# ZenHKD/ocr-vi-invoice

Hardware: AMD Instinct MI355X
Metric: invoice images/sec end-to-end (det+rec) (higher is better)
Workload: dtype f16x2

## Files before the change

include/ocrvi.h:

```cpp
#ifndef OCRVI_H
#define OCRVI_H

#include <stddef.h>
#include <stdint.h>

#ifdef __cplusplus
extern "C" {
#endif

#define OCRVI_OK 0
#define OCRVI_EINVAL (-1)
#define OCRVI_EHIP (-2)
#define OCRVI_ENOMEM (-3)
#define OCRVI_EBLOB (-4)
#define OCRVI_ERANGE (-5)

typedef enum { OCRVI_F32 = 0, OCRVI_BF16 = 1, OCRVI_F16 = 2, OCRVI_F16X2 = 3 } ocrvi_dtype;

const char* ocrvi_last_error(void);
int ocrvi_abi_version(void);

typedef struct ocrvi_det ocrvi_det;

typedef struct {
// ... 262 lines not shown
                        int C, int H, int W, int Co, int ksize, int sh, int sw, int groups, int act, int res_post, int out_f32, int in_place,
                        void* out_raw, float* out);
int ocrvi_test_gconv_plan(int dtype, int N, int C, int H, int W, int Co, int sh, int sw, int groups, int out_f32, int has_res, int n_cu,
                          int32_t plan[12]);
int ocrvi_test_conv3_halo_raw(int device, const float* x, const float* weight_host, const float* bias_host, int N, int C, int H, int W, int Co,
                              int act, void* out_raw, float* out);
int ocrvi_test_bneck_tail_raw(int device, const float* t1, const float* identity, const float* w2_host, const float* b2_host,
                              const float* w3_host, const float* b3_host, const float* w1_host, const float* b1_host, int N, int H, int W,
                              int no_phase_c, void* y_raw, void* t1n_raw, float* y_out, float* t1n_out);
int ocrvi_test_stem_pool_raw(int device, int dtype, const float* x, const float* weight_host, const float* bias_host, int N, int H, int W,
                             int fused, void* out_raw, float* out);
int ocrvi_test_halo_plan(int kind, int N, int C, int H, int W, int Co, int n_cu, int32_t plan[8]);
int ocrvi_test_stem_pool(int device, int dtype, const float* x, const float* weight_host, const float* bias_host, int N, int H, int W, int fused,
                         float* out, int iters, float* avg_ms);
int ocrvi_test_attention(int device, int dtype, const float* qkv, int B, int N, int heads, float* out, int iters,
                         float* avg_ms);

int ocrvi_test_mlp(int device, int dtype, float* x, const float* ln_g_host, const float* ln_b_host, const float* w1_host, const float* b1_host,
                   const float* w2_host, const float* b2_host, const float* next_g_host, const float* next_b_host, int want_xn, int M, int D,
                   float* xn_out, int iters, float* avg_ms);
int ocrvi_test_mlp_raw(int device, int dtype, float* x, const float* ln_g_host, const float* ln_b_host, const float* w1_host, const float* b1_host,
                       const float* w2_host, const float* b2_host, const float* next_g_host, const float* next_b_host, int M, int D, void* xn_raw,
                       float* xn_out, int iters, float* avg_ms);
int ocrvi_test_lin_x2(int device, const float* a, const float* weight_host, const float* bias_host, int M, int K, int N, int max_workgroups,
                      void* out_raw, float* out, int iters, float* avg_ms);
int ocrvi_test_pack_f16x2(const float* src, size_t n, void* dst, float* wscale);
int ocrvi_test_pack_stream(int kind, const float* w0, const float* w1, int d0, int d1, void* out, size_t cap, size_t* size, float scales[2]);
int ocrvi_test_swizzles(int32_t swz128_rows[64], int32_t swz_halo_rows[64]);
int ocrvi_test_persistent_grid(int ntile, int slots, int32_t* grid);

int ocrvi_test_layernorm(int device, int dtype, const float* x, int x_f32, int out_f32, const float* gamma_host, const float* beta_host,
                         int rows, int D, float* out);
int ocrvi_test_frm_vertical(int device, int dtype, const float* kv, const float* vq_host, int B, int H, int W, int D, float* out);
int ocrvi_test_asf(int device, int dtype, const float* p2, const float* p3, const float* p4, const float* p5, const float* w_host,
                   const float* b_host, int N, int H, int W, float* out);
int ocrvi_test_maxpool(int device, int dtype, const float* x, int N, int C, int H, int W, float* out);
int ocrvi_test_db_maps(int device, const float* bin_logits, const float* thresh_logits, float k, float* binary, float* thresh,
                       float* thresh_binary, size_t n);
int ocrvi_test_ctc_logsoftmax(int device, const float* logits, int ld, int B, int T, int C, float* log_probs, int32_t* argmax_ids);
int ocrvi_test_ctc_logsoftmax_conf(int device, const float* logits, int ld, int B, int T, int C, float* log_probs, int32_t* argmax_ids,
                                   float* best_lp);

int ocrvi_document_contour(const uint8_t* mask, int h, int w, int64_t stride, int32_t* quad , int32_t* found);
int ocrvi_document_contour_bits(const uint32_t* bits, int h, int w, int32_t* quad , int32_t* found);

#define OCRVI_DOC_AUTO 0
// ... 21 lines not shown
```

ocr_vi_invoice_amd/_lib.py:

```python
from __future__ import annotations

import ctypes as C
import os
from typing import Optional

_HERE = os.path.dirname(os.path.abspath(__file__))
LIB_PATH = os.environ.get("OCRVI_LIB") or os.path.join(_HERE, "lib", "libocrvi.so")

OCRVI_F32, OCRVI_BF16, OCRVI_F16, OCRVI_F16X2 = 0, 1, 2, 3
DTYPES = {"f32": OCRVI_F32, "fp32": OCRVI_F32, "float32": OCRVI_F32, "bf16": OCRVI_BF16, "bfloat16": OCRVI_BF16,
          "f16": OCRVI_F16, "fp16": OCRVI_F16, "float16": OCRVI_F16,
          "f16x2": OCRVI_F16X2}
ABI_VERSION = 5

EXPORTS = [
    "ocrvi_last_error", "ocrvi_abi_version",
    "ocrvi_det_create", "ocrvi_det_destroy", "ocrvi_det_workspace_bytes", "ocrvi_det_forward", "ocrvi_det_debug_features",
    "ocrvi_rec_create", "ocrvi_rec_destroy", "ocrvi_rec_workspace_bytes", "ocrvi_rec_forward", "ocrvi_rec_debug_features",
    "ocrvi_ctc_greedy", "ocrvi_normalize_u8", "ocrvi_resize_u8", "ocrvi_crop_resize_normalize", "ocrvi_db_postprocess", "ocrvi_db_boxes_batch",
    "ocrvi_unclip_polygon", "ocrvi_db_components_workspace_bytes", "ocrvi_db_components", "ocrvi_db_boxes_batch_sparse",
    "ocrvi_test_deform_conv", "ocrvi_test_offset_conv", "ocrvi_test_conv", "ocrvi_test_gemm", "ocrvi_test_attention", "ocrvi_test_mlp", "ocrvi_test_stem_pool", "ocrvi_test_pack_f16x2",
    "ocrvi_prof_enable", "ocrvi_prof_reset", "ocrvi_prof_report",
    "ocrvi_det_status", "ocrvi_rec_status", "ocrvi_range_reset", "ocrvi_range_flag",
    "ocrvi_resize_normalize_pages", "ocrvi_crop_resize_normalize_pages", "ocrvi_db_boxes_pages",
    "ocrvi_det_binary_workspace_bytes", "ocrvi_det_forward_binary",
    "ocrvi_four_point_transform", "ocrvi_warp_perspective_u8", "ocrvi_warp_perspective_pages",
    "ocrvi_test_layernorm", "ocrvi_test_frm_vertical", "ocrvi_test_asf", "ocrvi_test_maxpool", "ocrvi_test_db_maps", "ocrvi_test_ctc_logsoftmax",
    "ocrvi_det_eval_workspace_bytes", "ocrvi_det_eval", "ocrvi_ctc_loss", "ocrvi_edit_distance",
    "ocrvi_test_deform_conv_res",
    "ocrvi_enhance_init", "ocrvi_enhance_tables", "ocrvi_enhance_workspace_bytes", "ocrvi_enhance_u8",
    "ocrvi_rgb_to_lab_u8", "ocrvi_lab_to_rgb_u8", "ocrvi_clahe_lab_u8", "ocrvi_nlm_lab_u8", "ocrvi_sharpen_u8",
    "ocrvi_min_area_quads", "ocrvi_quad_crops", "ocrvi_crop_quad_resize_normalize_pages", "ocrvi_crop_quad_resize_normalize",
    "ocrvi_jpeg_info", "ocrvi_jpeg_parse", "ocrvi_jpeg_table_entry", "ocrvi_jpeg_decode_pages",
    "ocrvi_test_conv_res", "ocrvi_test_db_tail",
    "ocrvi_db_target_jobs", "ocrvi_db_target_maps", "ocrvi_resize_normalize_pad_pages",
    "ocrvi_test_mlp_raw", "ocrvi_test_lin_x2", "ocrvi_test_pack_stream", "ocrvi_test_swizzles", "ocrvi_test_persistent_grid",
    "ocrvi_test_bneck_tail",
    "ocrvi_jpeg_quant_tables", "ocrvi_jpeg_encode_header", "ocrvi_jpeg_encode_sizes", "ocrvi_jpeg_encode_table_entry", "ocrvi_jpeg_encode_pages",
    "ocrvi_test_gemm_raw", "ocrvi_test_ring_plan",
    "ocrvi_overlay_segments", "ocrvi_overlay_pages",
    "ocrvi_test_deform_conv_raw", "ocrvi_test_dcn_plan",
    "ocrvi_test_conv_raw", "ocrvi_test_gconv_plan",
    "ocrvi_png_info", "ocrvi_png_parse", "ocrvi_png_table_entry", "ocrvi_png_plan", "ocrvi_png_decode_pages",
    "ocrvi_png_encode_sizes", "ocrvi_png_encode_table_entry", "ocrvi_png_encode_pages", "ocrvi_test_png_code_lengths",
    "ocrvi_document_contour", "ocrvi_document_contour_bits", "ocrvi_doc_working_size", "ocrvi_doc_mask_sizes", "ocrvi_doc_mask_pages",
    "ocrvi_doc_grey_u8", "ocrvi_doc_smooth_u8", "ocrvi_doc_histogram", "ocrvi_doc_otsu", "ocrvi_doc_mask_bits",
    "ocrvi_rec_forward_conf", "ocrvi_ctc_greedy_conf", "ocrvi_test_ctc_logsoftmax_conf",
    "ocrvi_test_conv3_halo_raw", "ocrvi_test_bneck_tail_raw", "ocrvi_test_stem_pool_raw", "ocrvi_test_halo_plan",
    "ocrvi_ctc_beam_workspace_bytes", "ocrvi_ctc_beam",
]
PAGE_ENTRY = 4
DET_EVAL_RECORD_BYTES = 104
DET_EVAL_INT_SLOTS = ("tp", "fp", "fn", "positive_count", "negatives", "negative_count")
DET_EVAL_F64_SLOTS = ("pos_bce", "topk_bce", "dice_inter", "pred_mask", "gt_mask", "l1_num", "thresh_mask")
CTC_LOSS_MAX_TARGET = 1024
EDIT_DISTANCE_MAX_LEN = 2048
CTC_BEAM_MAX = 64
CTC_BEAM_MAX_T = 1024
CLAHE_WORKSPACE_BYTES = 16384
# ... 99 lines not shown
    lib.ocrvi_test_offset_conv.argtypes = [i32, i32, f32p, vp, vp, i32, i32, i32, i32, i32, f32p, i32, C.POINTER(C.c_float)]
    lib.ocrvi_test_conv.argtypes = [i32, i32, f32p, vp, vp, i32, i32, i32, i32, i32, i32, i32, i32, i32, i32, f32p, i32,
                                    C.POINTER(C.c_float)]
    lib.ocrvi_test_conv_res.argtypes = [i32, i32, f32p, vp, vp, f32p, i32, i32, i32, i32, i32, i32, i32, i32, f32p, i32, C.POINTER(C.c_float)]
    lib.ocrvi_test_bneck_tail.argtypes = [i32, f32p, f32p, vp, vp, vp, vp, vp, vp, i32, i32, i32, i32, f32p, f32p, i32, C.POINTER(C.c_float)]
    lib.ocrvi_test_db_tail.argtypes = [i32, i32, f32p, vp, vp, vp, vp, vp, vp, vp, vp, i32, i32, i32, i32, i32, f32p, f32p, i32,
                                       C.POINTER(C.c_float)]
    lib.ocrvi_test_gemm.argtypes = [i32, i32, f32p, vp, vp, f32p, i32, i32, i32, i32, i32, i32, f32p, i32, C.POINTER(C.c_float)]
    lib.ocrvi_test_gemm_raw.argtypes = [i32, i32, f32p, vp, vp, f32p, i32, i32, i32, i32, i32, i32, vp, f32p]
    lib.ocrvi_test_ring_plan.argtypes = [i32, i32, i32, i32, i32, i32, i32, i32, C.POINTER(C.c_int32)]
    lib.ocrvi_test_deform_conv_raw.argtypes = [i32, i32, f32p, f32p, f32p, vp, vp, f32p, i32, i32, i32, i32, i32, i32, i32, vp, f32p]
    lib.ocrvi_test_dcn_plan.argtypes = [i32, i32, i32, i32, i32, i32, i32, i32, C.POINTER(C.c_int32)]
    lib.ocrvi_test_conv_raw.argtypes = [i32, i32, f32p, vp, vp, f32p] + [i32] * 13 + [vp, f32p]
    lib.ocrvi_test_gconv_plan.argtypes = [i32] * 12 + [C.POINTER(C.c_int32)]
    lib.ocrvi_test_stem_pool.argtypes = [i32, i32, f32p, vp, vp, i32, i32, i32, i32, f32p, i32, C.POINTER(C.c_float)]
    lib.ocrvi_test_conv3_halo_raw.argtypes = [i32, f32p, vp, vp, i32, i32, i32, i32, i32, i32, vp, f32p]
    lib.ocrvi_test_bneck_tail_raw.argtypes = [i32, f32p, f32p, vp, vp, vp, vp, vp, vp, i32, i32, i32, i32, vp, vp, f32p, f32p]
    lib.ocrvi_test_stem_pool_raw.argtypes = [i32, i32, f32p, vp, vp, i32, i32, i32, i32, vp, f32p]
    lib.ocrvi_test_halo_plan.argtypes = [i32] * 7 + [C.POINTER(C.c_int32)]
    lib.ocrvi_test_attention.argtypes = [i32, i32, f32p, i32, i32, i32, f32p, i32, C.POINTER(C.c_float)]
    lib.ocrvi_test_mlp.argtypes = [i32, i32, f32p, vp, vp, vp, vp, vp, vp, vp, vp, i32, i32, i32, f32p, i32, C.POINTER(C.c_float)]
    lib.ocrvi_test_lin_x2.argtypes = [i32, f32p, vp, vp, i32, i32, i32, i32, vp, f32p, i32, C.POINTER(C.c_float)]
    lib.ocrvi_test_mlp_raw.argtypes = [i32, i32, f32p, vp, vp, vp, vp, vp, vp, vp, vp, i32, i32, vp, f32p, i32, C.POINTER(C.c_float)]
    lib.ocrvi_test_pack_f16x2.argtypes = [f32p, sz, vp, C.POINTER(C.c_float)]
    lib.ocrvi_test_pack_stream.argtypes = [i32, vp, vp, i32, i32, vp, sz, C.POINTER(sz), C.POINTER(C.c_float)]
    lib.ocrvi_test_swizzles.argtypes = [C.POINTER(C.c_int32), C.POINTER(C.c_int32)]
    lib.ocrvi_test_persistent_grid.argtypes = [i32, i32, C.POINTER(C.c_int32)]
    lib.ocrvi_test_layernorm.argtypes = [i32, i32, f32p, i32, i32, vp, vp, i32, i32, f32p]
    lib.ocrvi_test_frm_vertical.argtypes = [i32, i32, f32p, vp, i32, i32, i32, i32, f32p]
    lib.ocrvi_test_asf.argtypes = [i32, i32, f32p, f32p, f32p, f32p, vp, vp, i32, i32, i32, f32p]
    lib.ocrvi_test_maxpool.argtypes = [i32, i32, f32p, i32, i32, i32, i32, f32p]
    lib.ocrvi_test_db_maps.argtypes = [i32, f32p, f32p, C.c_float, f32p, f32p, f32p, sz]
    lib.ocrvi_test_ctc_logsoftmax.argtypes = [i32, f32p, i32, i32, i32, i32, f32p, i32p]
    lib.ocrvi_det_eval_workspace_bytes.argtypes = [i32, i32, i32, C.POINTER(sz)]
    lib.ocrvi_det_eval.argtypes = [i32, f32p, f32p, f32p, f32p, f32p, f32p, f32p, f32p, i32, i32, i32, C.c_double, vp, vp, sz, vp]
    lib.ocrvi_ctc_loss.argtypes = [i32, f32p, i32, i32, i32, i32p, i32, i32p, i32p, i32, vp, vp]
    lib.ocrvi_edit_distance.argtypes = [i32, i32p, i32, i32p, i32p, i32, i32p, i32, i32p, vp]
    lib.ocrvi_ctc_beam_workspace_bytes.argtypes = [i32, i32, i32, i32, C.POINTER(sz)]
    lib.ocrvi_ctc_beam.argtypes = [i32, f32p, i32, i32, i32, i32, i32, i32, i32p, i32p, vp, vp, sz, vp]
    lib.ocrvi_enhance_init.argtypes = [i32]
    lib.ocrvi_enhance_tables.argtypes = [vp, sz, C.POINTER(sz)]
    lib.ocrvi_enhance_workspace_bytes.argtypes = [i32, i32, C.POINTER(sz)]
    lib.ocrvi_enhance_u8.argtypes = [i32, vp, i32, i32, vp, vp, sz, vp]
    for name in ("ocrvi_rgb_to_lab_u8", "ocrvi_lab_to_rgb_u8", "ocrvi_nlm_lab_u8", "ocrvi_sharpen_u8"):
        getattr(lib, name).argtypes = [i32, vp, i32, i32, vp, vp]
    lib.ocrvi_clahe_lab_u8.argtypes = [i32, vp, i32, i32, vp, vp, sz, vp]
# ... 92 lines not shown
```

ocr_vi_invoice_amd/csrc/gemm_ring.h:

```cpp
#pragma once
#include "conv_gemm.h"

namespace ocrvi {

__device__ __forceinline__ void glds16(const char* sbase, unsigned voff, unsigned lds_dst) {
    unsigned keep;
    asm volatile("s_mov_b32 %0, m0\n\ts_mov_b32 m0, %3\n\ts_nop 0\n\tglobal_load_lds_dwordx4 %1, %2\n\ts_mov_b32 m0, %0"
                 : "=&s"(keep)
                 : "v"(voff), "s"(sbase), "s"(lds_dst)
                 : "memory");
}
__device__ __forceinline__ void glds16_sc1(const char* sbase, unsigned voff, unsigned lds_dst) {
    unsigned keep;
    asm volatile("s_mov_b32 %0, m0\n\ts_mov_b32 m0, %3\n\ts_nop 0\n\tglobal_load_lds_dwordx4 %1, %2 sc1\n\ts_mov_b32 m0, %0"
                 : "=&s"(keep)
                 : "v"(voff), "s"(sbase), "s"(lds_dst)
                 : "memory");
}
__device__ __forceinline__ void glds16v(const void* gsrc, unsigned lds_dst) {
    unsigned keep;
    asm volatile("s_mov_b32 %0, m0\n\ts_mov_b32 m0, %2\n\ts_nop 0\n\tglobal_load_lds_dwordx4 %1, off\n\ts_mov_b32 m0, %0"
                 : "=&s"(keep)
                 : "v"(gsrc), "s"(lds_dst)
                 : "memory");
}
__device__ __forceinline__ const char* uniform_ptr(const char* p) {
    const unsigned long long v = (unsigned long long)p;
    const unsigned lo = __builtin_amdgcn_readfirstlane((unsigned)v), hi = __builtin_amdgcn_readfirstlane((unsigned)(v >> 32));
    return (const char*)(((unsigned long long)hi << 32) | lo);
}
template <int N> __device__ __forceinline__ void wait_vm_barrier() {
    asm volatile("s_waitcnt vmcnt(%0)\n\ts_barrier" ::"n"(N) : "memory");
}

typedef unsigned int u32x4 __attribute__((ext_vector_type(4)));
__device__ __forceinline__ void gload16(u32x4& dst, const void* gsrc) {
    asm volatile("global_load_dwordx4 %0, %1, off" : "=v"(dst) : "v"(gsrc) : "memory");
}
__device__ __forceinline__ void gload16s(u32x4& dst, const char* sbase, unsigned voff) {
    asm volatile("global_load_dwordx4 %0, %1, %2" : "=v"(dst) : "v"(voff), "s"(sbase) : "memory");
}
template <int N> __device__ __forceinline__ void wait_vm_only() { asm volatile("s_waitcnt vmcnt(%0)" ::"n"(N) : "memory"); }
__device__ __forceinline__ void bind16(u32x4& r) { asm volatile("" : "+v"(r)); }
__device__ __forceinline__ uint4 lds16(const char* p) { return *(const uint4*)p; }

template <int I> struct IC { static constexpr int value = I; };

template <typename T, int BM, int NW, int SPS, bool F32O, bool C3 = false, int BN = 128, bool PROF = false, int ACT = -1>
__global__ __launch_bounds__(NW * 64, NW / 4) void gemm_ring_kernel(const ConvParams p) {
    constexpr int EPC = TypeInfo<T>::EPC, BKE = 8 * EPC;
    static_assert(BN == 128 || BN == 64, "column tile");
    constexpr int WN = BN / 64, WM = NW / WN, TM = BM / WM, TN = 64, MI = TM / 16, NI = 4;
    constexpr int STAGE = (BM + BN) * 128;
    constexpr int NSTAGE = 3, AHEAD = NSTAGE - 1;
    constexpr int NA = BM / 8 / NW, NB = BN / 8 / NW;
    constexpr int G = NA + NB;
    constexpr int NGRP = MI / SPS;
    static_assert(MI % SPS == 0, "slice group size must divide the wave's row blocks");
    constexpr int SG = F32O ? SPS * 4 : SPS * 2;
    static_assert(G + SG < 64, "vmcnt is a 6-bit counter");
    extern __shared__ __attribute__((aligned(16))) char smem[];
    const unsigned lds0 = (unsigned)(size_t)(__attribute__((address_space(3))) char*)smem;

    const int tid = threadIdx.x, lane = tid & 63;
// ... 516 lines not shown
```

ocr_vi_invoice_amd/csrc/kernels.h:

```cpp
#pragma once
#include "common.h"

namespace ocrvi {

int k_nchw3_to_nhwc4_pad(int dtype, const float* x, void* y, int N, int H, int W, int pad_t, int pad_l, int Hp, int Wp, hipStream_t s);
int k_maxpool3x3s2(int dtype, const void* x, void* y, int N, int H, int W, int C, hipStream_t s);
bool stem_pool_eligible(int dtype, int cout, int Kp, int KH, int H, int W);
int k_stem_pool(int dtype, const void* xpad, const void* w, const float* bias, float wscale, void* y, int N, int H, int W, int Hp, int Wp,
                hipStream_t s);
struct StemPoolPlan {
    int tyN, txN, total;
    int grid;
    int tiles_min, tiles_max;
};
StemPoolPlan stem_pool_plan(int N, int H, int W, int n_cu);
int k_layernorm(int dtype, const void* x, int x_f32, void* out, int out_f32, const float* gamma, const float* beta, int rows, int D,
                hipStream_t s);
bool mlp_fused_eligible(int dtype, int D);
bool mlp_x2_eligible(int dtype, int D);
void pack_mlp_x2_stream(const float* w1, const float* w2, int D, std::vector<char>& out);
int k_mlp_x2(float* x, void* xn, const float* ln_g, const float* ln_b, const float* next_g, const float* next_b, const void* wstream, const float* b1,
             const float* b2, int M, int D, hipStream_t s);
void pack_mlp_stream(const float* w1, const float* w2, int D, int dtype, std::vector<char>& out);
bool lin_x2_eligible(int dtype, int K, int N);
void pack_lin_x2_stream(const float* w, int N, int K, std::vector<char>& out);
int k_lin_x2(const void* a, const void* wstream, const float* bias, void* out, int M, int K, int N, hipStream_t s, int max_workgroups = 0);
int k_mlp_fused(int dtype, float* x, void* xn, const float* ln_g, const float* ln_b, const float* next_g, const float* next_b, const void* wstream,
                const float* b1, const float* b2, int M, int D, hipStream_t s);
int k_cast_from_f32(int dtype, const float* x, void* y, size_t n, hipStream_t s);
int k_nhwc_to_nchw_f32(int dtype, const void* x, float* y, int N, int H, int W, int C, int ld, int coff, hipStream_t s);

int k_attention(int dtype, const void* qkv, void* out, int B, int N, int heads, hipStream_t s, void* scratch = nullptr);
size_t attention_scratch_bytes(int dtype, int B, int N, int heads);
int k_frm_vertical(int dtype, const void* kv, const float* vq, void* out, int B, int H, int W, int D, hipStream_t s);

int k_asf(int dtype, const void* p2, const void* p3, const void* p4, const void* p5, const float* w, const float* b, float* scratch, void* out,
          int N, int H, int W, hipStream_t s);
size_t asf_scratch_bytes(int N, int H, int W);
int k_db_maps(const float* bin_logits, const float* thresh_logits, float k, float* binary, float* thresh, float* thresh_binary, size_t n,
              hipStream_t s);

int k_ctc_logsoftmax_argmax(const float* logits, int ld, float* log_probs, int32_t* argmax_ids, int B, int T, int C, hipStream_t s);
int k_ctc_argmax_tbc(const float* log_probs, int32_t* argmax_ids, int B, int T, int C, hipStream_t s);
int k_ctc_collapse(const int32_t* argmax_ids, int32_t* ids, int32_t* lens, int B, int T, int blank, hipStream_t s);
int k_ctc_logsoftmax_argmax_conf(const float* logits, int ld, float* log_probs, int32_t* argmax_ids, float* best_lp, int B, int T, int C,
// ... 7 lines not shown
```

ocr_vi_invoice_amd/csrc/lin_x2.hip:

```cpp
#include <stdlib.h>
#include <string.h>

#include "gemm_ring.h"
#include "kernels.h"
#include "weight_pack.h"

namespace ocrvi {
OCRVI_RANGE_FLAG_TU()

struct LinX2Params {
    const char* a = nullptr;
    const char* wstream = nullptr;
    const float* bias = nullptr;
    void* out = nullptr;
    unsigned out_bytes = 0;
    int M = 0, N = 0;
};

constexpr int LIN_X2_MAX_N = 2048;

template <int K, int R>
__global__ __launch_bounds__(512, 2) void lin_x2_kernel(const LinX2Params p) {
    typedef f16x2_t T;
    typedef Mma<T>::u4v U;
// ... 31 lines not shown
    auto issue_unit = [&]() {
        const char* src = wbase + (size_t)prod_mod * UNIT + wave * 1024;
        const unsigned dst = lds0 + prod_slot * UNIT + wave * 1024;
#pragma unroll
        for (int j = 0; j < IPW; ++j) glds16(src + j * (NWV * 1024), (unsigned)lane * 16u, __builtin_amdgcn_readfirstlane(dst + j * (NWV * 1024)));
        prod_slot = prod_slot + 1 == R ? 0 : prod_slot + 1;
        prod_mod = prod_mod + 1 == NU ? 0 : prod_mod + 1;
    };
    auto next_unit = [&]() -> const char* {
        wait_vm_barrier<(PF - 1) * IPW + NST>();
        issue_unit();
        const char* s = smem + cons_slot * UNIT;
        cons_slot = cons_slot + 1 == R ? 0 : cons_slot + 1;
        return s;
    };
    for (int i = 0; i < PF; ++i) issue_unit();
    const int sw = swz128(lr);
    const int fo0 = ((2 * g) ^ sw) << 4, fo1 = ((2 * g + 1) ^ sw) << 4;
    unsigned long long range_mask = 0;
    const __amdgpu_buffer_rsrc_t orsrc = __builtin_amdgcn_make_buffer_rsrc(p.out, 0, (int)p.out_bytes, 0x00020000);
    constexpr unsigned OOB = 0xfffffff0u;
    const unsigned ldo_b = (unsigned)p.N * 4u;

    for (int t = 0; t < my_tiles; ++t) {
        const int tile = (int)blockIdx.x + t * G;
        const int tok = tile * 128 + wave * 16 + q_tok;
        U xH[KS], xL[KS];
        {
            const char* xr = p.a + (size_t)min(tok, p.M - 1) * (K * 4) + 32 * q_g;
            uint4 c[KS][2];
#pragma unroll
            for (int ks = 0; ks < KS; ++ks) {
                c[ks][0] = *(const uint4*)(xr + 128 * ks);
                c[ks][1] = *(const uint4*)(xr + 128 * ks + 16);
            }
            auto mv = [&](unsigned v) { return (unsigned)__builtin_amdgcn_ds_bpermute(to_mfma, (int)v); };
#pragma unroll
            for (int ks = 0; ks < KS; ++ks) {
                const uint4 c0 = make_uint4(mv(c[ks][0].x), mv(c[ks][0].y), mv(c[ks][0].z), mv(c[ks][0].w));
                const uint4 c1 = make_uint4(mv(c[ks][1].x), mv(c[ks][1].y), mv(c[ks][1].z), mv(c[ks][1].w));
                Mma<T>::regroup(c0, c1, xH[ks], xL[ks]);
            }
        }
        wait_vm_only<0>();
        const unsigned row_b = tok < p.M ? (unsigned)tok * ldo_b + 16u * (unsigned)q_g : OOB;

        for (int u = 0; u < NU; ++u) {
            const char* const U1 = next_unit();
            f32x4 acc[2];
            {
                int l = threadIdx.x;
                asm volatile("" : "+v"(l));
                const float* bp = c_b + 32 * u + 4 * ((l & 63) >> 4);
                const float4 b0 = *(const float4*)bp, b1 = *(const float4*)(bp + 16);
                acc[0] = (f32x4){b0.x, b0.y, b0.z, b0.w};
                acc[1] = (f32x4){b1.x, b1.y, b1.z, b1.w};
            }
            constexpr int P1 = 2;
            uint4 wr[P1 + 1][2][2];
            auto rd1 = [&](int ks, int set) {
#pragma unroll
                for (int a = 0; a < 2; ++a) {
                    const char* r = U1 + (ks * 32 + 16 * a + lr) * 128;
                    wr[set][a][0] = *(const uint4*)(r + fo0);
                    wr[set][a][1] = *(const uint4*)(r + fo1);
                }
            };
#pragma unroll
            for (int i = 0; i < P1; ++i) rd1(i, i);
            __builtin_amdgcn_sched_barrier(0);
#pragma unroll
            for (int ks = 0; ks < KS; ++ks) {
                if (ks + P1 < KS) rd1(ks + P1, (ks + P1) % (P1 + 1));
                __builtin_amdgcn_sched_barrier(0);
#pragma unroll
                for (int a = 0; a < 2; ++a)
                    Mma<T>::three(Mma<T>::as_u4v(wr[ks % (P1 + 1)][a][0]), Mma<T>::as_u4v(wr[ks % (P1 + 1)][a][1]), xH[ks], xL[ks], acc[a]);
                __builtin_amdgcn_sched_barrier(0);
            }
            const unsigned off = row_b != OOB ? row_b + 128u * (unsigned)u : OOB;
#pragma unroll
            for (int a = 0; a < 2; ++a) {
                const float v[4] = {unscale<T>(acc[a][0], ws), unscale<T>(acc[a][1], ws), unscale<T>(acc[a][2], ws), unscale<T>(acc[a][3], ws)};
                range_mask |= f16x2_out_of_range(v);
                const uint4 e = Chunk<T>::pack(v);
                auto mv = [&](unsigned x) { return (unsigned)__builtin_amdgcn_ds_bpermute(to_quad, (int)x); };
                __builtin_amdgcn_raw_buffer_store_b128((u32x4){mv(e.x), mv(e.y), mv(e.z), mv(e.w)}, orsrc, off != OOB ? off + 64u * a : OOB, 0, 0);
            }
        }
    }
    wait_vm_only<0>();
    f16x2_raise(range_mask);
}

bool lin_x2_eligible(int dtype, int K, int N) {
    return mlp_x2_eligible(dtype, K) && (K == 256 || K == 384) && N > 0 && N % 32 == 0 && N <= LIN_X2_MAX_N;
}

void pack_lin_x2_stream(const float* w, int N, int K, std::vector<char>& out) {
    const int KS = K / 32, NU = N / 32;
// ... 41 lines not shown
```

ocr_vi_invoice_amd/csrc/mlp_x2.hip:

```cpp
#include <stdlib.h>
#include <string.h>

#include "gemm_ring.h"
#include "kernels.h"
#include "weight_pack.h"

namespace ocrvi {
OCRVI_RANGE_FLAG_TU()

struct MlpX2Params {
    float* x = nullptr;
    void* xn = nullptr;
    const float* ln_g = nullptr;
    const float* ln_b = nullptr;
    const float* next_g = nullptr;
    const float* next_b = nullptr;
    const char* wstream = nullptr;
    const float* b1 = nullptr;
    const float* b2 = nullptr;
    int M = 0;
};

template <int D, int R, int TB, bool SPLIT>
__global__ __launch_bounds__(512 / TB, TB == 2 ? 1 : 2) void mlp_x2_kernel(const MlpX2Params p) {
// ... 28 lines not shown
        c_g[i] = p.ln_g[i];
        c_be[i] = p.ln_b[i];
        c_ng[i] = next_ln ? p.next_g[i] : 1.f;
        c_nb[i] = next_ln ? p.next_b[i] : 0.f;
    }
    const float* const tail = (const float*)(p.wstream + (size_t)(NCH + 1) * 2 * W1B);
    const float ws1 = tail[0], ws2 = tail[1];
    __syncthreads();

    const int ntiles = (p.M + 127) >> 7;
    const int G = gridDim.x;
    const int my_tiles = (ntiles - (int)blockIdx.x + G - 1) / G;

    const char* const wbase = uniform_ptr(p.wstream);
    int prod_slot = 0, prod_mod = 0, cons_slot = 0;
    auto issue_unit = [&]() {
        const char* src = wbase + (size_t)prod_mod * UNIT + wave * 1024;
        const unsigned dst = lds0 + prod_slot * UNIT + wave * 1024;
#pragma unroll
        for (int j = 0; j < IPW; ++j) glds16(src + j * (NWV * 1024), (unsigned)lane * 16u, __builtin_amdgcn_readfirstlane(dst + j * (NWV * 1024)));
        prod_slot = prod_slot + 1 == R ? 0 : prod_slot + 1;
        prod_mod = prod_mod + 1 == NU ? 0 : prod_mod + 1;
    };
    auto next_unit = [&]() -> const char* {
        wait_vm_barrier<(PF - 1) * IPW>();
        issue_unit();
        const char* s = smem + cons_slot * UNIT;
        cons_slot = cons_slot + 1 == R ? 0 : cons_slot + 1;
        return s;
    };
    for (int i = 0; i < PF; ++i) issue_unit();
    const int sw = swz128(lr);
    const int fo0 = ((2 * g) ^ sw) << 4, fo1 = ((2 * g + 1) ^ sw) << 4;
    unsigned long long range_mask = 0;

    for (int t = 0; t < my_tiles; ++t) {
        const int tile = (int)blockIdx.x + t * G;
        const int tok0 = tile * 128 + wave * (16 * TB);
        U xH[KS][TB], xL[KS][TB];
#pragma unroll
        for (int b = 0; b < TB; ++b) {
            float xv[KS][8];
            const int tok = min(tok0 + 16 * b + lr, p.M - 1);
            const float* xr = p.x + (size_t)tok * D + 8 * g;
#pragma unroll
            for (int ks = 0; ks < KS; ++ks) {
                const float4 v0 = *(const float4*)(xr + 32 * ks), v1 = *(const float4*)(xr + 32 * ks + 4);
                xv[ks][0] = v0.x; xv[ks][1] = v0.y; xv[ks][2] = v0.z; xv[ks][3] = v0.w;
                xv[ks][4] = v1.x; xv[ks][5] = v1.y; xv[ks][6] = v1.z; xv[ks][7] = v1.w;
            }
            float sum = 0.f;
#pragma unroll
            for (int ks = 0; ks < KS; ++ks)
#pragma unroll
                for (int e = 0; e < 8; ++e) sum += xv[ks][e];
            sum += __shfl_xor(sum, 16);
            sum += __shfl_xor(sum, 32);
            const float mean = sum / (float)D;
            float sq = 0.f;
#pragma unroll
            for (int ks = 0; ks < KS; ++ks)
#pragma unroll
                for (int e = 0; e < 8; ++e) { const float d = xv[ks][e] - mean; sq += d * d; }
            sq += __shfl_xor(sq, 16);
            sq += __shfl_xor(sq, 32);
            const float rstd = rsqrtf(sq / (float)D + 1e-5f);
#pragma unroll
            for (int ks = 0; ks < KS; ++ks) {
                float o[8];
#pragma unroll
                for (int q = 0; q < 2; ++q) {
                    const float4 gv = *(const float4*)(c_g + 32 * ks + 8 * g + 4 * q), bv = *(const float4*)(c_be + 32 * ks + 8 * g + 4 * q);
                    o[4 * q] = (xv[ks][4 * q] - mean) * rstd * gv.x + bv.x;
                    o[4 * q + 1] = (xv[ks][4 * q + 1] - mean) * rstd * gv.y + bv.y;
                    o[4 * q + 2] = (xv[ks][4 * q + 2] - mean) * rstd * gv.z + bv.z;
                    o[4 * q + 3] = (xv[ks][4 * q + 3] - mean) * rstd * gv.w + bv.w;
                }
                const uint4 c0 = Chunk<T>::pack(o), c1 = Chunk<T>::pack(o + 4);
                Mma<T>::regroup(c0, c1, xH[ks][b], xL[ks][b]);
            }
        }
        wait_vm_only<0>();

        f32x4 acc2[NB2][TB];
#pragma unroll
        for (int a = 0; a < NB2; ++a)
#pragma unroll
            for (int b = 0; b < TB; ++b) acc2[a][b] = (f32x4){0.f, 0.f, 0.f, 0.f};

        f32x4 hacc[2][TB], hprev[2][TB];
        constexpr int NV = 8 * TB;
        auto gelu_vals = [&](int i0, int i1, const float* bp) {
#pragma unroll
            for (int i = i0; i < i1; ++i) {
                const int b = i >> 3, a = (i >> 2) & 1, r = i & 3;
                hprev[a][b][r] = gelu_erf(hprev[a][b][r] * ws1 + bp[16 * a + r]);
            }
        };
        auto g1 = [&](const char* U1, bool with_gelu, const float* bv) {
#pragma unroll
            for (int a = 0; a < 2; ++a)
#pragma unroll
                for (int b = 0; b < TB; ++b) hacc[a][b] = (f32x4){0.f, 0.f, 0.f, 0.f};
            constexpr int P1 = TB == 2 ? 1 : 2;
            uint4 wr[P1 + 1][2][2];
// ... 44 lines not shown
                Mma<T>::regroup(c0, c1, hH[b], hL[b]);
            }
            __builtin_amdgcn_sched_barrier(0);
#pragma unroll
            for (int grp = 0; grp < NG; ++grp) {
                if (grp + PFG < NG) rd2(grp + PFG, (grp + PFG) % (PFG + 1));
                __builtin_amdgcn_sched_barrier(0);
#pragma unroll
                for (int i = 0; i < GB; ++i)
#pragma unroll
                    for (int b = 0; b < TB; ++b)
                        Mma<T>::three(Mma<T>::as_u4v(w2r[grp % (PFG + 1)][i][0]), Mma<T>::as_u4v(w2r[grp % (PFG + 1)][i][1]), hH[b], hL[b], acc2[grp * GB + i][b]);
                __builtin_amdgcn_sched_barrier(0);
            }
        };
        auto keep = [&]() {
#pragma unroll
            for (int a = 0; a < 2; ++a)
#pragma unroll
                for (int b = 0; b < TB; ++b) hprev[a][b] = hacc[a][b];
        };
        auto second = [&](const char* U1) -> const char* {
            if constexpr (SPLIT) {
                return next_unit();
            } else {
                return U1 + W1B;
            }
        };
        auto bias_of = [&](int c) {
            int l = threadIdx.x;
            asm volatile("" : "+v"(l));
            return c_b1 + 32 * c + 4 * ((l & 63) >> 4);
        };
        {
            const char* const U1 = next_unit();
            g1(U1, false, bias_of(0));
            (void)second(U1);
        }
        keep();
        for (int k = 1; k < NCH; ++k) {
            const char* const U1 = next_unit();
            g1(U1, true, bias_of(k - 1));
            g2(second(U1));
            keep();
        }
        {
            const char* const U1 = next_unit();
            gelu_vals(0, NV, bias_of(NCH - 1));
            g2(second(U1));
        }

        const int pn_tok = lane >> 2, pn_g = lane & 3;
        const int pn_src = 4 * (16 * pn_g + pn_tok);
#pragma unroll
        for (int b = 0; b < TB; ++b) {
#pragma unroll
            for (int a = 0; a < NB2; ++a)
#pragma unroll
                for (int r = 0; r < 4; ++r)
                    acc2[a][b][r] = __int_as_float(__builtin_amdgcn_ds_bpermute(pn_src, __float_as_int(acc2[a][b][r])));
            const int tok = tok0 + 16 * b + pn_tok;
            const bool ok = tok < p.M;
            float* xr = p.x + (size_t)(ok ? tok : 0) * D + 4 * pn_g;
            float sum = 0.f;
            float4 rvs[NB2];
#pragma unroll
            for (int a = 0; a < NB2; ++a) rvs[a] = *(const float4*)(xr + 16 * a);
#pragma unroll
            for (int a = 0; a < NB2; ++a) {
                const float4 bv2 = *(const float4*)(c_b2 + 16 * a + 4 * pn_g);
                const float4 rv = rvs[a];
                f32x4 v = acc2[a][b];
                v[0] = v[0] * ws2 + bv2.x + rv.x; v[1] = v[1] * ws2 + bv2.y + rv.y; v[2] = v[2] * ws2 + bv2.z + rv.z; v[3] = v[3] * ws2 + bv2.w + rv.w;
                acc2[a][b] = v;
                if (ok) *(float4*)(xr + 16 * a) = make_float4(v[0], v[1], v[2], v[3]);
                sum += v[0] + v[1] + v[2] + v[3];
            }
            if (p.xn) {
                float mean = 0.f, rstd = 1.f;
                if (next_ln) {
                    sum += __shfl_xor(sum, 1);
                    sum += __shfl_xor(sum, 2);
                    mean = sum / (float)D;
                    float sq = 0.f;
#pragma unroll
                    for (int a = 0; a < NB2; ++a)
#pragma unroll
                        for (int r = 0; r < 4; ++r) { const float d = acc2[a][b][r] - mean; sq += d * d; }
                    sq += __shfl_xor(sq, 1);
                    sq += __shfl_xor(sq, 2);
                    rstd = rsqrtf(sq / (float)D + 1e-5f);
                }
// ... 25 lines not shown
    const size_t units = (size_t)(NCH + 1) * (KS * 32 + D) * 128;
    out.assign(units + 8, 0);
    char* dst = out.data();
    float v[32];
    for (int k = 0; k <= NCH; ++k) {
        for (int ks = 0; ks < KS; ++ks)
            for (int r = 0; r < 32; ++r, dst += 128) {
                for (int e = 0; e < 32; ++e) v[e] = k < NCH ? w1[(size_t)(32 * k + r) * D + 32 * ks + e] : 0.f;
                f16x2_put_row(v, s1, swz128(ks * 32 + r), dst);
            }
        for (int n = 0; n < D; ++n, dst += 128) {
            for (int pos = 0; pos < 32; ++pos) {
                const int g = pos >> 3, j = pos & 7;
                v[pos] = k >= 1 ? w2[(size_t)n * H4 + 32 * (k - 1) + 16 * (j >> 2) + 4 * g + (j & 3)] : 0.f;
            }
            f16x2_put_row(v, s2, swz128(n), dst);
        }
    }
    const float tail[2] = {1.0f / s1, 1.0f / s2};
    memcpy(out.data() + units, tail, 8);
}

template <int D, int R, int TB, bool SPLIT>
static int launch_mlp_x2(const MlpX2Params& p, hipStream_t s) {
    const int smem = R * (SPLIT ? 128 : 256) * D + 9 * D * 4;
    auto kern = mlp_x2_kernel<D, R, TB, SPLIT>;
    OCRVI_TRY(ensure_max_smem((const void*)kern, smem));
    int n_cu = 0;
    OCRVI_TRY(device_cus(&n_cu));
    const int ntiles = (p.M + 127) / 128;
    const int grid = persistent_grid(ntiles, n_cu);
    hipLaunchKernelGGL(kern, dim3(grid), dim3(512 / TB), smem, s, p);
    OCRVI_HIP(hipGetLastError());
    return OCRVI_OK;
}

int k_mlp_x2(float* x, void* xn, const float* ln_g, const float* ln_b, const float* next_g, const float* next_b, const void* wstream, const float* b1,
             const float* b2, int M, int D, hipStream_t s) {
    OCRVI_CHECK((D == 128 || D == 256 || D == 384) && x && ln_g && ln_b && wstream && b1 && b2 && M > 0 && M < (1 << 24), OCRVI_EINVAL,
                "mlp_x2: bad argument (D %d, M %d)", D, M);
    MlpX2Params p;
    p.x = x; p.xn = xn; p.ln_g = ln_g; p.ln_b = ln_b; p.next_g = next_g; p.next_b = next_b; p.wstream = (const char*)wstream; p.b1 = b1; p.b2 = b2; p.M = M;
    char tag[64];
    snprintf(tag, sizeof(tag), "mlp_fused_d%d_f16x2", D);
    ProfScope ps(tag, 2.0 * M * 8.0 * D * D, (double)M * D * (8.0 + (xn ? 4.0 : 0.0)) + 8.0 * D * D * 4.0, s);
    if (D == 128) return launch_mlp_x2<128, 4, 1, false>(p, s);
    if (D == 256) return launch_mlp_x2<256, 2, 1, false>(p, s);
    return launch_mlp_x2<384, 3, 2, true>(p, s);
}

}
```

Measured before the change: 331.5.

## Prefetch next tile's activation rows during GEMM in f16x2 MLP and linear kernels

In the persistent f16x2 linear and fused-MLP kernels, the activation rows for the next tile are now loaded into registers while the current tile's last weight unit is still in MMA work. The MLP kernel also issues its residual loads early, and counts outstanding loads with explicit vmcnt waits. This hides global-load latency at tile boundaries. The cost is more register pressure and delicate waitcnt bookkeeping. A max_workgroups test hook and a test export are also added.

New measurement: 331.4, median of 2. No clear change (-0.0%).

```diff
diff --git a/include/ocrvi.h b/include/ocrvi.h
--- a/include/ocrvi.h
+++ b/include/ocrvi.h
@@ -308,6 +308,9 @@
 int ocrvi_test_mlp_raw(int device, int dtype, float* x, const float* ln_g_host, const float* ln_b_host, const float* w1_host, const float* b1_host,
                        const float* w2_host, const float* b2_host, const float* next_g_host, const float* next_b_host, int M, int D, void* xn_raw,
                        float* xn_out, int iters, float* avg_ms);
+int ocrvi_test_mlp_x2_wg(int device, float* x, const float* ln_g_host, const float* ln_b_host, const float* w1_host, const float* b1_host,
+                         const float* w2_host, const float* b2_host, const float* next_g_host, const float* next_b_host, int want_xn, int M, int D,
+                         int max_workgroups, void* xn_raw, float* xn_out, int iters, float* avg_ms);
 int ocrvi_test_lin_x2(int device, const float* a, const float* weight_host, const float* bias_host, int M, int K, int N, int max_workgroups,
                       void* out_raw, float* out, int iters, float* avg_ms);
 int ocrvi_test_pack_f16x2(const float* src, size_t n, void* dst, float* wscale);
diff --git a/ocr_vi_invoice_amd/_lib.py b/ocr_vi_invoice_amd/_lib.py
--- a/ocr_vi_invoice_amd/_lib.py
+++ b/ocr_vi_invoice_amd/_lib.py
@@ -34,7 +34,7 @@
     "ocrvi_jpeg_info", "ocrvi_jpeg_parse", "ocrvi_jpeg_table_entry", "ocrvi_jpeg_decode_pages",
     "ocrvi_test_conv_res", "ocrvi_test_db_tail",
     "ocrvi_db_target_jobs", "ocrvi_db_target_maps", "ocrvi_resize_normalize_pad_pages",
-    "ocrvi_test_mlp_raw", "ocrvi_test_lin_x2", "ocrvi_test_pack_stream", "ocrvi_test_swizzles", "ocrvi_test_persistent_grid",
+    "ocrvi_test_mlp_raw", "ocrvi_test_mlp_x2_wg", "ocrvi_test_lin_x2", "ocrvi_test_pack_stream", "ocrvi_test_swizzles", "ocrvi_test_persistent_grid",
     "ocrvi_test_bneck_tail",
     "ocrvi_jpeg_quant_tables", "ocrvi_jpeg_encode_header", "ocrvi_jpeg_encode_sizes", "ocrvi_jpeg_encode_table_entry", "ocrvi_jpeg_encode_pages",
     "ocrvi_test_gemm_raw", "ocrvi_test_ring_plan",
@@ -180,6 +180,7 @@
     lib.ocrvi_test_mlp.argtypes = [i32, i32, f32p, vp, vp, vp, vp, vp, vp, vp, vp, i32, i32, i32, f32p, i32, C.POINTER(C.c_float)]
     lib.ocrvi_test_lin_x2.argtypes = [i32, f32p, vp, vp, i32, i32, i32, i32, vp, f32p, i32, C.POINTER(C.c_float)]
     lib.ocrvi_test_mlp_raw.argtypes = [i32, i32, f32p, vp, vp, vp, vp, vp, vp, vp, vp, i32, i32, vp, f32p, i32, C.POINTER(C.c_float)]
+    lib.ocrvi_test_mlp_x2_wg.argtypes = [i32, f32p, vp, vp, vp, vp, vp, vp, vp, vp, i32, i32, i32, i32, vp, f32p, i32, C.POINTER(C.c_float)]
     lib.ocrvi_test_pack_f16x2.argtypes = [f32p, sz, vp, C.POINTER(C.c_float)]
     lib.ocrvi_test_pack_stream.argtypes = [i32, vp, vp, i32, i32, vp, sz, C.POINTER(sz), C.POINTER(C.c_float)]
     lib.ocrvi_test_swizzles.argtypes = [C.POINTER(C.c_int32), C.POINTER(C.c_int32)]
diff --git a/ocr_vi_invoice_amd/csrc/gemm_ring.h b/ocr_vi_invoice_amd/csrc/gemm_ring.h
--- a/ocr_vi_invoice_amd/csrc/gemm_ring.h
+++ b/ocr_vi_invoice_amd/csrc/gemm_ring.h
@@ -40,6 +40,30 @@
 __device__ __forceinline__ void gload16s(u32x4& dst, const char* sbase, unsigned voff) {
     asm volatile("global_load_dwordx4 %0, %1, %2" : "=v"(dst) : "v"(voff), "s"(sbase) : "memory");
 }
+template <int OFF> __device__ __forceinline__ void gload16o(u32x4& dst, const void* gsrc) {
+    asm volatile("global_load_dwordx4 %0, %1, off offset:%2" : "=v"(dst) : "v"(gsrc), "n"(OFF) : "memory");
+}
+template <int KS, int I = 0> __device__ __forceinline__ void gload_row(u32x4 (&dst)[KS][2], const void* row) {
+    if constexpr (I < KS) {
+        gload16o<128 * I>(dst[I][0], row);
+        gload16o<128 * I + 16>(dst[I][1], row);
+        gload_row<KS, I + 1>(dst, row);
+    }
+}
+template <int N, int STRIDE, int I = 0> __device__ __forceinline__ void gload_strided(u32x4 (&dst)[N], const void* p) {
+    if constexpr (I < N) {
+        gload16o<STRIDE * I>(dst[I], p);
+        gload_strided<N, STRIDE, I + 1>(dst, p);
+    }
+}
+template <int K0, int N, int NA, int I = 0> __device__ __forceinline__ void gload_row_split(u32x4 (&lo)[NA], u32x4 (&hi)[NA], const void* row) {
+    if constexpr (I < N) {
+        gload16o<128 * (K0 + I)>(lo[I], row);
+        gload16o<128 * (K0 + I) + 16>(hi[I], row);
+        gload_row_split<K0, N, NA, I + 1>(lo, hi, row);
+    }
+}
+constexpr int vm_count(int n) { return n < 63 ? n : 63; }
 template <int N> __device__ __forceinline__ void wait_vm_only() { asm volatile("s_waitcnt vmcnt(%0)" ::"n"(N) : "memory"); }
 __device__ __forceinline__ void bind16(u32x4& r) { asm volatile("" : "+v"(r)); }
 __device__ __forceinline__ uint4 lds16(const char* p) { return *(const uint4*)p; }
diff --git a/ocr_vi_invoice_amd/csrc/kernels.h b/ocr_vi_invoice_amd/csrc/kernels.h
--- a/ocr_vi_invoice_amd/csrc/kernels.h
+++ b/ocr_vi_invoice_amd/csrc/kernels.h
@@ -20,7 +20,7 @@
 bool mlp_x2_eligible(int dtype, int D);
 void pack_mlp_x2_stream(const float* w1, const float* w2, int D, std::vector<char>& out);
 int k_mlp_x2(float* x, void* xn, const float* ln_g, const float* ln_b, const float* next_g, const float* next_b, const void* wstream, const float* b1,
-             const float* b2, int M, int D, hipStream_t s);
+             const float* b2, int M, int D, hipStream_t s, int max_workgroups = 0);
 void pack_mlp_stream(const float* w1, const float* w2, int D, int dtype, std::vector<char>& out);
 bool lin_x2_eligible(int dtype, int K, int N);
 void pack_lin_x2_stream(const float* w, int N, int K, std::vector<char>& out);
diff --git a/ocr_vi_invoice_amd/csrc/lin_x2.hip b/ocr_vi_invoice_amd/csrc/lin_x2.hip
--- a/ocr_vi_invoice_amd/csrc/lin_x2.hip
+++ b/ocr_vi_invoice_amd/csrc/lin_x2.hip
@@ -77,31 +77,50 @@
     constexpr unsigned OOB = 0xfffffff0u;
     const unsigned ldo_b = (unsigned)p.N * 4u;
 
+    constexpr int NSEP = KS <= 8 ? KS : 8, NREU = KS - NSEP;
+    U xH[KS], xL[KS];
+    u32x4 pf[NSEP][2];
+    auto row_of = [&](int t) {
+        const int tok = ((int)blockIdx.x + t * G) * 128 + wave * 16 + q_tok;
+        return p.a + (size_t)min(tok, p.M - 1) * (K * 4) + 32 * q_g;
+    };
+    if (my_tiles > 0) {
+        const char* xr = row_of(0);
+        gload_row<NSEP>(pf, xr);
+        gload_row_split<NSEP, NREU>(xH, xL, xr);
+    }
+    wait_vm_only<0>();
+
     for (int t = 0; t < my_tiles; ++t) {
         const int tile = (int)blockIdx.x + t * G;
         const int tok = tile * 128 + wave * 16 + q_tok;
-        U xH[KS], xL[KS];
+        const bool has_next = t + 1 < my_tiles;
+        wait_vm_only<NST>();
         {
-            const char* xr = p.a + (size_t)min(tok, p.M - 1) * (K * 4) + 32 * q_g;
-            uint4 c[KS][2];
-#pragma unroll
-            for (int ks = 0; ks < KS; ++ks) {
-                c[ks][0] = *(const uint4*)(xr + 128 * ks);
-                c[ks][1] = *(const uint4*)(xr + 128 * ks + 16);
-            }
             auto mv = [&](unsigned v) { return (unsigned)__builtin_amdgcn_ds_bpermute(to_mfma, (int)v); };
-#pragma unroll
-            for (int ks = 0; ks < KS; ++ks) {
-                const uint4 c0 = make_uint4(mv(c[ks][0].x), mv(c[ks][0].y), mv(c[ks][0].z), mv(c[ks][0].w));
-                const uint4 c1 = make_uint4(mv(c[ks][1].x), mv(c[ks][1].y), mv(c[ks][1].z), mv(c[ks][1].w));
-                Mma<T>::regroup(c0, c1, xH[ks], xL[ks]);
+            auto frag = [&](const u32x4& r0, const u32x4& r1, U& H, U& L) {
+                const uint4 c0 = make_uint4(mv(r0[0]), mv(r0[1]), mv(r0[2]), mv(r0[3]));
+                const uint4 c1 = make_uint4(mv(r1[0]), mv(r1[1]), mv(r1[2]), mv(r1[3]));
+                Mma<T>::regroup(c0, c1, H, L);
+            };
+#pragma unroll
+            for (int i = 0; i < NREU; ++i) {
+                bind16(xH[i]); bind16(xL[i]);
+                frag(xH[i], xL[i], xH[NSEP + i], xL[NSEP + i]);
+            }
+#pragma unroll
+            for (int ks = 0; ks < NSEP; ++ks) {
+                bind16(pf[ks][0]); bind16(pf[ks][1]);
+                frag(pf[ks][0], pf[ks][1], xH[ks], xL[ks]);
             }
         }
-        wait_vm_only<0>();
         const unsigned row_b = tok < p.M ? (unsigned)tok * ldo_b + 16u * (unsigned)q_g : OOB;
 
+        const char* const xr_next = row_of(has_next ? t + 1 : t);
         for (int u = 0; u < NU; ++u) {
             const char* const U1 = next_unit();
+            const bool fetch = has_next && u == NU - 1;
+            if (fetch) gload_row<NSEP>(pf, xr_next);
             f32x4 acc[2];
             {
                 int l = threadIdx.x;
@@ -131,6 +150,7 @@
 #pragma unroll
                 for (int a = 0; a < 2; ++a)
                     Mma<T>::three(Mma<T>::as_u4v(wr[ks % (P1 + 1)][a][0]), Mma<T>::as_u4v(wr[ks % (P1 + 1)][a][1]), xH[ks], xL[ks], acc[a]);
+                if (NREU > 0 && ks == NREU && fetch) gload_row_split<NSEP, NREU>(xH, xL, xr_next);
                 __builtin_amdgcn_sched_barrier(0);
             }
             const unsigned off = row_b != OOB ? row_b + 128u * (unsigned)u : OOB;
diff --git a/ocr_vi_invoice_amd/csrc/mlp_x2.hip b/ocr_vi_invoice_amd/csrc/mlp_x2.hip
--- a/ocr_vi_invoice_amd/csrc/mlp_x2.hip
+++ b/ocr_vi_invoice_amd/csrc/mlp_x2.hip
@@ -74,8 +74,8 @@
         prod_slot = prod_slot + 1 == R ? 0 : prod_slot + 1;
         prod_mod = prod_mod + 1 == NU ? 0 : prod_mod + 1;
     };
-    auto next_unit = [&]() -> const char* {
-        wait_vm_barrier<(PF - 1) * IPW>();
+    auto next_unit = [&](auto extra) -> const char* {
+        wait_vm_barrier<vm_count((PF - 1) * IPW + decltype(extra)::value)>();
         issue_unit();
         const char* s = smem + cons_slot * UNIT;
         cons_slot = cons_slot + 1 == R ? 0 : cons_slot + 1;
@@ -86,21 +86,57 @@
     const int fo0 = ((2 * g) ^ sw) << 4, fo1 = ((2 * g + 1) ^ sw) << 4;
     unsigned long long range_mask = 0;
 
+    constexpr bool AHEAD = TB == 1;
+    u32x4 pf[KS][2];
+    auto row_of = [&](int t, int b) {
+        int l = threadIdx.x;
+        asm volatile("" : "+v"(l));
+        const int tok = min(((int)blockIdx.x + t * G) * 128 + wave * (16 * TB) + 16 * b + (l & 15), p.M - 1);
+        return p.x + (size_t)tok * D + 8 * ((l & 63) >> 4);
+    };
+    auto drop_rows = [&]() {
+#pragma unroll
+        for (int ks = 0; ks < KS; ++ks) { asm volatile("" : "=v"(pf[ks][0])); asm volatile("" : "=v"(pf[ks][1])); }
+    };
+    if constexpr (AHEAD) {
+        if (my_tiles > 0) gload_row<KS>(pf, row_of(0, 0)); else drop_rows();
+        wait_vm_only<0>();
+    }
+    constexpr int ST_TILE = NB2, ST_TILE_XN = 2 * NB2;
+
     for (int t = 0; t < my_tiles; ++t) {
         const int tile = (int)blockIdx.x + t * G;
         const int tok0 = tile * 128 + wave * (16 * TB);
+        const bool has_next = t + 1 < my_tiles;
+        float xvs[TB][KS][8];
+        if constexpr (AHEAD) {
+            if (t > 0) {
+                if (p.xn) wait_vm_only<vm_count(ST_TILE_XN)>();
+                else wait_vm_only<vm_count(ST_TILE)>();
+            }
+#pragma unroll
+            for (int ks = 0; ks < KS; ++ks) {
+                bind16(pf[ks][0]); bind16(pf[ks][1]);
+#pragma unroll
+                for (int e = 0; e < 8; ++e) xvs[0][ks][e] = __uint_as_float(pf[ks][e >> 2][e & 3]);
+            }
+        } else {
+#pragma unroll
+            for (int b = 0; b < TB; ++b) {
+                const float* xr = row_of(t, b);
+#pragma unroll
+                for (int ks = 0; ks < KS; ++ks) {
+                    const float4 v0 = *(const float4*)(xr + 32 * ks), v1 = *(const float4*)(xr + 32 * ks + 4);
+                    xvs[b][ks][0] = v0.x; xvs[b][ks][1] = v0.y; xvs[b][ks][2] = v0.z; xvs[b][ks][3] = v0.w;
+                    xvs[b][ks][4] = v1.x; xvs[b][ks][5] = v1.y; xvs[b][ks][6] = v1.z; xvs[b][ks][7] = v1.w;
+                }
+            }
+        }
         U xH[KS][TB], xL[KS][TB];
 #pragma unroll
-        for (int b = 0; b < TB; ++b) {
-            float xv[KS][8];
-            const int tok = min(tok0 + 16 * b + lr, p.M - 1);
-            const float* xr = p.x + (size_t)tok * D + 8 * g;
-#pragma unroll
-            for (int ks = 0; ks < KS; ++ks) {
-                const float4 v0 = *(const float4*)(xr + 32 * ks), v1 = *(const float4*)(xr + 32 * ks + 4);
-                xv[ks][0] = v0.x; xv[ks][1] = v0.y; xv[ks][2] = v0.z; xv[ks][3] = v0.w;
-                xv[ks][4] = v1.x; xv[ks][5] = v1.y; xv[ks][6] = v1.z; xv[ks][7] = v1.w;
-            }
+        for (int bb = 0; bb < TB; ++bb) {
+            const int b = bb;
+            float (&xv)[KS][8] = xvs[b];
             float sum = 0.f;
 #pragma unroll
             for (int ks = 0; ks < KS; ++ks)
@@ -132,7 +168,7 @@
                 Mma<T>::regroup(c0, c1, xH[ks][b], xL[ks][b]);
             }
         }
-        wait_vm_only<0>();
+        if constexpr (!AHEAD) wait_vm_only<0>();
 
         f32x4 acc2[NB2][TB];
 #pragma unroll
@@ -223,7 +259,7 @@
         };
         auto second = [&](const char* U1) -> const char* {
             if constexpr (SPLIT) {
-                return next_unit();
+                return next_unit(IC<0>());
             } else {
                 return U1 + W1B;
             }
@@ -233,26 +269,33 @@
             asm volatile("" : "+v"(l));
             return c_b1 + 32 * c + 4 * ((l & 63) >> 4);
         };
+        const int pn_tok = lane >> 2, pn_g = lane & 3;
+        const int pn_src = 4 * (16 * pn_g + pn_tok);
+        const int pn_tok0 = tok0 + pn_tok;
+        u32x4 rva[NB2];
         {
-            const char* const U1 = next_unit();
+            const char* const U1 = !AHEAD || t == 0 ? next_unit(IC<0>()) : p.xn ? next_unit(IC<ST_TILE_XN>()) : next_unit(IC<ST_TILE>());
             g1(U1, false, bias_of(0));
             (void)second(U1);
         }
         keep();
         for (int k = 1; k < NCH; ++k) {
-            const char* const U1 = next_unit();
+            const char* const U1 = next_unit(IC<0>());
             g1(U1, true, bias_of(k - 1));
             g2(second(U1));
             keep();
         }
         {
-            const char* const U1 = next_unit();
+            const char* const U1 = next_unit(IC<0>());
             gelu_vals(0, NV, bias_of(NCH - 1));
-            g2(second(U1));
-        }
-
-        const int pn_tok = lane >> 2, pn_g = lane & 3;
-        const int pn_src = 4 * (16 * pn_g + pn_tok);
+            const char* const U2 = second(U1);
+            if constexpr (AHEAD) gload_strided<NB2, 64>(rva, p.x + (size_t)(pn_tok0 < p.M ? pn_tok0 : 0) * D + 4 * pn_g);
+            g2(U2);
+            if constexpr (AHEAD) {
+                if (has_next) gload_row<KS>(pf, row_of(t + 1, 0)); else drop_rows();
+            }
+        }
+
 #pragma unroll
         for (int b = 0; b < TB; ++b) {
 #pragma unroll
@@ -265,10 +308,19 @@
             float* xr = p.x + (size_t)(ok ? tok : 0) * D + 4 * pn_g;
             float sum = 0.f;
             float4 rvs[NB2];
-#pragma unroll
-            for (int a = 0; a < NB2; ++a) rvs[a] = *(const float4*)(xr + 16 * a);
+            if constexpr (!AHEAD) {
+#pragma unroll
+                for (int a = 0; a < NB2; ++a) rvs[a] = *(const float4*)(xr + 16 * a);
+            } else if (!has_next) {
+                wait_vm_only<0>();
+            }
 #pragma unroll
             for (int a = 0; a < NB2; ++a) {
+                if constexpr (AHEAD) {
+                    wait_vm_only<vm_count(NB2 - 1 + 2 * KS)>();
+                    bind16(rva[a]);
+                    rvs[a] = make_float4(__uint_as_float(rva[a][0]), __uint_as_float(rva[a][1]), __uint_as_float(rva[a][2]), __uint_as_float(rva[a][3]));
+                }
                 const float4 bv2 = *(const float4*)(c_b2 + 16 * a + 4 * pn_g);
                 const float4 rv = rvs[a];
                 f32x4 v = acc2[a][b];
@@ -340,21 +392,21 @@
 }
 
 template <int D, int R, int TB, bool SPLIT>
-static int launch_mlp_x2(const MlpX2Params& p, hipStream_t s) {
+static int launch_mlp_x2(const MlpX2Params& p, int max_workgroups, hipStream_t s) {
     const int smem = R * (SPLIT ? 128 : 256) * D + 9 * D * 4;
     auto kern = mlp_x2_kernel<D, R, TB, SPLIT>;
     OCRVI_TRY(ensure_max_smem((const void*)kern, smem));
     int n_cu = 0;
     OCRVI_TRY(device_cus(&n_cu));
     const int ntiles = (p.M + 127) / 128;
-    const int grid = persistent_grid(ntiles, n_cu);
+    const int grid = persistent_grid(ntiles, max_workgroups > 0 ? std::min(n_cu, max_workgroups) : n_cu);
     hipLaunchKernelGGL(kern, dim3(grid), dim3(512 / TB), smem, s, p);
     OCRVI_HIP(hipGetLastError());
     return OCRVI_OK;
 }
 
 int k_mlp_x2(float* x, void* xn, const float* ln_g, const float* ln_b, const float* next_g, const float* next_b, const void* wstream, const float* b1,
-             const float* b2, int M, int D, hipStream_t s) {
+             const float* b2, int M, int D, hipStream_t s, int max_workgroups) {
     OCRVI_CHECK((D == 128 || D == 256 || D == 384) && x && ln_g && ln_b && wstream && b1 && b2 && M > 0 && M < (1 << 24), OCRVI_EINVAL,
                 "mlp_x2: bad argument (D %d, M %d)", D, M);
     MlpX2Params p;
@@ -362,9 +414,9 @@
     char tag[64];
     snprintf(tag, sizeof(tag), "mlp_fused_d%d_f16x2", D);
     ProfScope ps(tag, 2.0 * M * 8.0 * D * D, (double)M * D * (8.0 + (xn ? 4.0 : 0.0)) + 8.0 * D * D * 4.0, s);
-    if (D == 128) return launch_mlp_x2<128, 4, 1, false>(p, s);
-    if (D == 256) return launch_mlp_x2<256, 2, 1, false>(p, s);
-    return launch_mlp_x2<384, 3, 2, true>(p, s);
-}
-
-}
+    if (D == 128) return launch_mlp_x2<128, 4, 1, false>(p, max_workgroups, s);
+    if (D == 256) return launch_mlp_x2<256, 2, 1, false>(p, max_workgroups, s);
+    return launch_mlp_x2<384, 3, 2, true>(p, max_workgroups, s);
+}
+
+}
```
